# apache/datafusion-comet

Hardware: NVIDIA H100
Metric: rows/sec on TPC-H Q1 filter+agg (higher is better)
Workload: dtype i128

## Files before the change

### datafusion-comet_b200/csrc/abi.cpp

```cpp
#include "../../include/comet_b200.h"

#include "abi_internal.h"
#include "parquet_kernels.h"
#include "exec_internal.h"
#include "jit.h"
#include "plan.h"
#include "proto_wire.h"

#include <cstring>
#include <functional>
#include <map>
#include <mutex>

using namespace cb200;

namespace {

struct CtxRes {
    cudaStream_t stream;
    int* d_err;
    int* h_err;
    cudaEvent_t ev0, ev1;
};
std::mutex g_pool_mu;
// ... 27 lines not shown
    {
        struct DevInfo { int major = 0, minor = 0, sms = 0; bool known = false; };
        static DevInfo info[64];
        static std::mutex info_mu;
        std::lock_guard<std::mutex> lk(info_mu);
        if (ctx.device < 0 || ctx.device >= 64) throw ExecError(CB200_ERR_CUDA, "", "device ordinal out of range");
        DevInfo& di = info[ctx.device];
        if (!di.known) {
            cuda_check(cudaDeviceGetAttribute(&di.major, cudaDevAttrComputeCapabilityMajor, ctx.device), "cudaDeviceGetAttribute");
            cuda_check(cudaDeviceGetAttribute(&di.minor, cudaDevAttrComputeCapabilityMinor, ctx.device), "cudaDeviceGetAttribute");
            cuda_check(cudaDeviceGetAttribute(&di.sms, cudaDevAttrMultiProcessorCount, ctx.device), "cudaDeviceGetAttribute");
            di.known = true;
        }
        if (di.major != 9 || di.minor != 0) throw ExecError(CB200_ERR_CUDA, "", "comet_b200 kernels are built for sm_90a; device is sm_" + std::to_string(di.major * 10 + di.minor));
        ctx.num_sms = di.sms;
    }
    {
        std::lock_guard<std::mutex> lk(g_pool_mu);
        auto& fl = g_pool[ctx.device];
        if (!fl.empty()) {
            CtxRes r = fl.back();
            fl.pop_back();
            ctx.stream = r.stream; ctx.d_err = r.d_err; ctx.h_err = r.h_err; ctx.ev0 = r.ev0; ctx.ev1 = r.ev1;
        }
    }
    if (!ctx.stream) {
        cuda_check(cudaStreamCreateWithFlags(&ctx.stream, cudaStreamNonBlocking), "cudaStreamCreate");
        cudaMemPool_t pool;
        if (cudaDeviceGetDefaultMemPool(&pool, ctx.device) == cudaSuccess) {
            unsigned long long keep = ~0ull;
            cudaMemPoolSetAttribute(pool, cudaMemPoolAttrReleaseThreshold, &keep);
        }
        cuda_check(cudaMalloc((void**)&ctx.d_err, 64), "cudaMalloc err");
        cuda_check(cudaMallocHost((void**)&ctx.h_err, 64), "cudaMallocHost err");
        cuda_check(cudaEventCreate(&ctx.ev0), "cudaEventCreate");
        cuda_check(cudaEventCreate(&ctx.ev1), "cudaEventCreate");
    }
    cuda_check(cudaMemsetAsync(ctx.d_err, 0, 64, ctx.stream), "memset err");
    set_alloc_stream(ctx.stream);
    p->root = build_exec(p->op, &ctx, &p->inputs);
    p->started = true;
}

DType dtype_from_ids(int type_id, int precision, int scale) {
    if (type_id < 0 || type_id > 13) throw Unsupported("type id " + std::to_string(type_id));
    DType d;
    d.id = (TypeId)type_id;
    d.precision = precision;
    d.scale = scale;
    return d;
}

}

extern "C" {

const char* cb200_version(void) { return "comet_b200 0.1.0 (sm_90a; reference apache/datafusion-comet 1.1.0 @2699f59b)"; }

int cb200_supports(const uint8_t* op_proto, size_t op_len, cb200_error* why) {
    return cb200_guarded(why, [&]() -> int {
        OperatorP op = decode_plan(op_proto, op_len);
        plan_kernels_for_build(op);
        return 1;
    }, 0);
}

cb200_plan* cb200_create_plan(const uint8_t* op_proto, size_t op_len, const uint8_t* cfg_proto, size_t cfg_len, struct ArrowArrayStream** inputs,
// ... 329 lines not shown
```

### datafusion-comet_b200/csrc/agg.cpp

```cpp
#include "exec_internal.h"
#include "../../include/comet_b200.h"

#include "aot_kernels.h"
#include "ranges.h"

#include <algorithm>
#include <mutex>

namespace cb200 {

static std::mutex g_profile_mu;
static std::map<std::string, std::vector<int>> g_range_profile;

void reset_range_profiles() {
    std::lock_guard<std::mutex> lk(g_profile_mu);
    g_range_profile.clear();
}

namespace {

enum class Strategy { Undecided, Dense, Table, Stream };
enum Level { SAFE = 0, TYPE = 1, TIGHT = 2 };
constexpr int DENSE_MAX_GROUPS = 64;

// ... 42 lines not shown
            for (int k = (int)cards.size() - 1; k >= 0; k--) {
                int cd = code[(size_t)k];
                if (has_null[(size_t)k] && cd == cards[(size_t)k] - 1) cd = new_cards[(size_t)k] - 1;
                ng += cd * mul;
                mul *= new_cards[(size_t)k];
            }
            memcpy(&newt[(size_t)ng * n_words * 2], &oldt[(size_t)g * n_words * 2], (size_t)n_words * 16);
        }
        totals = host_to_device(newt.data(), newt.size() * 8, ctx, "regroup H2D");
        groups = new_groups;
    }

    void finalize(ExecContext* ctx, const Kernel& last, cb::FinParams fp, bool ungrouped, const std::vector<DType>& schema,
                  const std::vector<DictionaryP>& key_dicts, Batch& out) const {
        TraceSpan ts("agg.finalize");
        const GeneratedKernel& g = last.g;
        const int ng = groups;
        fp.totals = (cb::u64*)totals->ptr;
        fp.n_groups = ng;
        std::vector<size_t> off_v, off_n;
        size_t total_bytes = 0;
        auto take = [&](size_t n) { size_t o = total_bytes; total_bytes += (n + 15) / 16 * 16; return o; };
        for (size_t i = 0; i < g.out_cols.size(); i++) { off_v.push_back(take((size_t)ng * g.out_bytes[i])); off_n.push_back(take((size_t)ng)); }
        size_t off_present = take((size_t)ng);
        auto dbuf = std::make_shared<DeviceBuf>(total_bytes);
        for (size_t i = 0; i < g.out_cols.size(); i++) {
            fp.out[i] = (cb::u8*)dbuf->ptr + off_v[i];
            fp.outv[i] = (cb::u8*)dbuf->ptr + off_n[i];
        }
        fp.present = (cb::u8*)dbuf->ptr + off_present;
        void* args[] = {&fp};
        cuda_check(cudaLaunchKernel((const void*)last.mod->kernel(g.finalize_entry), dim3((ng + 127) / 128), dim3(128), args, 0, ctx->stream), "finalize launch");
        ctx->kernel_launches++;
        std::vector<uint8_t> hbuf(total_bytes);
        cuda_check(cudaMemcpyAsync(hbuf.data(), dbuf->ptr, total_bytes, cudaMemcpyDeviceToHost, ctx->stream), "agg results D2H"); ctx->d2h_bytes += (int64_t)(total_bytes);
        ctx->check_device_errors();
        const uint8_t* pres = hbuf.data() + off_present;
        std::vector<int> rows;
        for (int gi = 0; gi < ng; gi++) if (ungrouped || pres[(size_t)gi]) rows.push_back(gi);
        out.n_rows = (int64_t)rows.size();
        out.cols.clear();
        for (size_t k = 0; k < key_dicts.size(); k++) {
            Column c;
            c.type = schema[k];
            c.on_host = true;
            bool any_null = false;
            std::vector<int> codes;
            for (int gi : rows) codes.push_back(decode_gid(gi, cards)[k]);
            c.h_valid.assign(rows.size(), 1);
            const bool is_bool = c.type.id == TypeId::Bool;
            if (!is_bool) c.h_offsets.push_back(0);
            for (size_t r = 0; r < rows.size(); r++) {
                const bool isnull = has_null[k] && codes[r] == cards[k] - 1;
                if (isnull) { c.h_valid[r] = 0; any_null = true; }
                if (is_bool) c.h_data.push_back(isnull ? 0 : (uint8_t)codes[r]);
                else {
                    if (!isnull) { const std::string& s = key_dicts[k]->values().at((size_t)codes[r]); c.h_data.insert(c.h_data.end(), s.begin(), s.end()); }
                    c.h_offsets.push_back((int32_t)c.h_data.size());
                }
            }
            if (!any_null) c.h_valid.clear();
            out.cols.push_back(c);
        }
        for (size_t i = 0; i < g.out_cols.size(); i++) {
            Column c;
            c.type = g.out_cols[i].type;
            c.on_host = true;
            int w = g.out_bytes[i];
            const uint8_t* all = hbuf.data() + off_v[i];
            const uint8_t* allv = hbuf.data() + off_n[i];
            c.h_data.resize(rows.size() * w);
            c.h_valid.resize(rows.size());
            bool any_null = false;
            for (size_t r = 0; r < rows.size(); r++) {
                memcpy(&c.h_data[r * w], &all[(size_t)rows[r] * w], (size_t)w);
                c.h_valid[r] = allv[(size_t)rows[r]];
                if (!c.h_valid[r]) any_null = true;
            }
            if (!any_null) c.h_valid.clear();
            out.cols.push_back(c);
        }
    }
};

struct IdRows {
    DeviceBufP hkey_of_gid, htotals, hflags;
    int64_t max_groups = 0;

    void ensure_flags(ExecContext* ctx) {
        if (hflags) return;
        hflags = std::make_shared<DeviceBuf>(sizeof(HashFlags));
        cuda_check(cudaMemsetAsync(hflags->ptr, 0, sizeof(HashFlags), ctx->stream), "memset hash flags");
    }
    void write_flags(ExecContext* ctx, const HashFlags& hf) {
        cuda_check(cudaMemcpyAsync(hflags->ptr, &hf, sizeof(hf), cudaMemcpyHostToDevice, ctx->stream), "write hash flags");
        cuda_check(cudaStreamSynchronize(ctx->stream), "flags sync");
    }
    int64_t read_flags(ExecContext* ctx, HashFlags& hf, int64_t cnt[GK]) {
        memset(&hf, 0, sizeof(hf));
        if (hflags) {
            cuda_check(cudaMemcpyAsync(&hf, hflags->ptr, sizeof(hf), cudaMemcpyDeviceToHost, ctx->stream), "read hash flags"); ctx->d2h_bytes += (int64_t)sizeof(hf);
            cuda_check(cudaStreamSynchronize(ctx->stream), "hash flags sync");
        }
// ... 269 lines not shown
        Kernel k{spec, generate_pipeline(spec), nullptr};
        k.mod = jit_get(k.g, true);
        if (have_totals() && k.g.key_words != key_words) throw ExecError(15, "", "internal: group key packing changed between launches");
        if (have_totals() && (k.g.n_words != n_words || k.g.word_kinds != word_kinds || k.g.role_words != role_words)) widen(k);
        n_words = k.g.n_words;
        word_kinds = k.g.word_kinds;
        role_words = k.g.role_words;
        key_words = k.g.key_words;
        return k;
    }

    void widen(const Kernel& k) {
        GeneratedKernel from;
        from.n_words = n_words;
        from.word_kinds = word_kinds;
        from.role_words = role_words;
        const std::vector<int> map = widen_word_map(from, k.g);
        if (map.empty()) throw ExecError(15, "", "internal: accumulator layout changed between launches");
        const bool is_dense = strategy == Strategy::Dense;
        DeviceBufP& t = is_dense ? dense.totals : rows.htotals;
        const size_t n_rows = is_dense ? (size_t)dense.groups : (size_t)rows.max_groups + 2;
        auto nt = std::make_shared<DeviceBuf>(n_rows * (size_t)k.g.n_words * 16);
        for (int w = 0; w < k.g.n_words; w++)
            cuda_check(cudaMemcpy2DAsync((char*)nt->ptr + (size_t)w * 16, (size_t)k.g.n_words * 16, (const char*)t->ptr + (size_t)map[(size_t)w] * 16,
                                         (size_t)n_words * 16, 16, n_rows, cudaMemcpyDeviceToDevice, ctx->stream), "widen totals");
        cuda_check(cudaStreamSynchronize(ctx->stream), "widen totals");
        t = nt;
    }

    void clear_vmask() {
        if (!vmask) vmask = std::make_shared<DeviceBuf>(CB_MAX_COLS * 16);
        cuda_check(cudaMemsetAsync(vmask->ptr, 0, CB_MAX_COLS * 16, ctx->stream), "memset vmask");
    }
    void copy_vmask(ValueMasks& masks) {
        cuda_check(cudaMemcpyAsync(masks, vmask->ptr, sizeof(ValueMasks), cudaMemcpyDeviceToHost, ctx->stream), "read value masks"); ctx->d2h_bytes += (int64_t)(sizeof(ValueMasks));
    }
    static std::vector<int> mask_bits(const PipelineSpec& spec, const ValueMasks& masks) {
        std::vector<int> seen(spec.cols.size(), -1);
        for (size_t i = 0; i < spec.cols.size(); i++) {
            if (!spec.cols[i].type.is_decimal()) continue;
            uint64_t lo = masks[2 * i], hi = masks[2 * i + 1];
            seen[i] = hi ? 64 + r_bitlen(hi) : r_bitlen(lo);
        }
        return seen;
    }
    void observe(const std::vector<int>& seen) {
        for (size_t i = 0; i < seen.size(); i++)
            if (seen[i] >= 0) observed_bits[(size_t)used_cols[i]] = std::max(observed_bits[(size_t)used_cols[i]], seen[i]);
    }

    int prepare_key(Batch& b, size_t k) {
        int ci = keys[k]->index;
        Column& c = b.cols[ci];
        if (c.type.id == TypeId::Bool) return 2;
        if (!c.type.is_string()) return -1;
        if (c.is_dict) {
            key_dicts[k] = c.dict;
            return (int)c.dict->values().size();
        }
        if (!dev_dicts[k]) {
            auto dd = std::make_shared<DevDict>();
            const int64_t cap = 1 << 16;
            const int max_codes = 4096;
            const int64_t bytes_cap = 1 << 20;
            auto alloc = [&](size_t n) { auto bfr = std::make_shared<DeviceBuf>(n); cuda_check(cudaMemsetAsync(bfr->ptr, 0, bfr->bytes, ctx->stream), "memset dict"); dd->bufs.push_back(bfr); return bfr->ptr; };
            dd->d.tags = (unsigned long long*)alloc((size_t)cap * 8);
            dd->d.slot_code = (int*)alloc((size_t)cap * 4);
            dd->d.capacity = cap;
            dd->d.n_codes = (int*)alloc(64);
            dd->d.bytes_used = (unsigned long long*)((char*)dd->d.n_codes + 16);
            dd->d.err = (int*)((char*)dd->d.n_codes + 32);
            dd->d.max_codes = max_codes;
            dd->d.code_off = (long long*)alloc((size_t)max_codes * 8);
            dd->d.code_len = (int*)alloc((size_t)max_codes * 4);
            dd->d.bytes = (unsigned char*)alloc((size_t)bytes_cap);
            dd->d.bytes_cap = bytes_cap;
            dev_dicts[k] = dd;
            key_dicts[k] = std::make_shared<Dictionary>();
        }
        DevDict& dd = *dev_dicts[k];
        if (!c.offsets || !c.chars) throw Unsupported("string key column without offsets/chars buffers");
        auto row_slot = std::make_shared<DeviceBuf>((size_t)b.n_rows * 4);
        auto codes = std::make_shared<DeviceBuf>((size_t)b.n_rows * 4);
        launch_dict_encode(dd.d, (const int*)c.offsets->ptr, (const unsigned char*)c.chars->ptr, c.validity ? (const unsigned char*)c.validity->ptr : nullptr,
                           b.n_rows, (int*)row_slot->ptr, (int*)codes->ptr, ctx->stream);
        ctx->kernel_launches += 2;
        int hdr[12];
        cuda_check(cudaMemcpyAsync(hdr, dd.d.n_codes, sizeof(hdr), cudaMemcpyDeviceToHost, ctx->stream), "dict header");
        cuda_check(cudaStreamSynchronize(ctx->stream), "dict encode");
        int n_codes = hdr[0], derr = hdr[8];
        if (derr & CB_DICT_FULL) throw Unsupported("plain Utf8 group key with more distinct values than the device dictionary holds (dictionary-encode the column)");
        if (derr & CB_DICT_COLLISION) throw ExecError(14, "", "64-bit hash collision between distinct group key strings");
        if (n_codes > dd.host_known) {
            std::vector<long long> off((size_t)n_codes);
            std::vector<int> len((size_t)n_codes);
            cuda_check(cudaMemcpy(off.data(), dd.d.code_off, (size_t)n_codes * 8, cudaMemcpyDeviceToHost), "dict offsets");
            cuda_check(cudaMemcpy(len.data(), dd.d.code_len, (size_t)n_codes * 4, cudaMemcpyDeviceToHost), "dict lengths");
            for (int i = dd.host_known; i < n_codes; i++) {
                std::string s((size_t)len[(size_t)i], '\0');
                if (len[(size_t)i]) cuda_check(cudaMemcpy(&s[0], dd.d.bytes + off[(size_t)i], (size_t)len[(size_t)i], cudaMemcpyDeviceToHost), "dict bytes");
                key_dicts[k]->append(s);
            }
            dd.host_known = n_codes;
        }
        c.data = codes;
        c.phys = Phys::I32;
        c.is_dict = true;
        c.dict = key_dicts[k];
        return n_codes;
    }

    void consume(Batch& b) {
        for (int ci : used_cols) if (b.cols[(size_t)ci].validity) col_nullable[(size_t)ci] = true;
        std::vector<int> nc(keys.size());
        std::vector<bool> hn(keys.size());
        for (size_t k = 0; k < keys.size(); k++) {
            int card = prepare_key(b, k);
            const Column& c = b.cols[keys[k]->index];
            hn[k] = key_has_null[k] || c.validity != nullptr;
            nc[k] = card < 0 ? -1 : std::max(card, 1) + (hn[k] ? 1 : 0);
            if (!dense.cards.empty() && nc[k] >= 0) nc[k] = std::max(nc[k], dense.cards[k]);
        }
        bool densifiable = true;
        for (int c : nc) if (c < 0) densifiable = false;
        int n_groups = 1;
        if (densifiable) for (int c : nc) { n_groups *= c; if (n_groups > 1 << 20) break; }
        const bool needs_hash = !ungrouped && (!densifiable || n_groups > DENSE_MAX_GROUPS);
        key_has_null = hn;
        if (observed_bits.empty()) observed_bits.assign(child->schema.size(), -1);
        if (strategy == Strategy::Undecided || (strategy == Strategy::Dense && needs_hash)) {
            if (strategy == Strategy::Dense) {
                leave_dense();
                ctx->agg_strategies |= CB200_AGG_MIGRATED;
// ... 65 lines not shown
            while (r0 < row1 && launch_one(b, r0, std::min(row1, r0 + max_rows), n_groups, k, lv)) r0 += max_rows;
            if (r0 >= row1) return;
            if (lv == SAFE) throw ExecError(15, "", "internal: value-mask validation failed without assumptions");
            lv = lv == TIGHT ? TYPE : SAFE;
            row0 = r0;
        }
    }

    bool launch_one(Batch& b, int64_t r0, int64_t r1, int n_groups, const Kernel& k, Level lv) {
        cudaStream_t st = ctx->stream;
        size_t tot_bytes = (size_t)n_groups * n_words * 16;
        if (!have_totals()) {
            dense.totals = std::make_shared<DeviceBuf>(tot_bytes);
            dense.groups = n_groups;
        }
        if (!dense.spill || dense.spill->bytes < tot_bytes) {
            dense.spill = std::make_shared<DeviceBuf>(tot_bytes);
            cuda_check(cudaMemsetAsync(dense.spill->ptr, 0, dense.spill->bytes, st), "memset spill");
        }
        clear_vmask();
        cb::PipeParams p;
        fill_inputs(p, b, k.g.tile, r0, r1);
        bind_str_masks(p, k.spec, b);
        int grid = grid_for(ctx, p.n_tiles);
        size_t part_bytes = (size_t)grid * tot_bytes;
        if (!dense.partials || dense.partials->bytes < part_bytes) dense.partials = std::make_shared<DeviceBuf>(part_bytes);
        p.n_groups = n_groups;
        for (size_t i = 0; i < dense.cards.size() && i < CB_MAX_KEYS; i++) p.key_card[i] = dense.cards[i];
        p.partials = (cb::u8*)dense.partials->ptr;
        p.spill = (cb::u64*)dense.spill->ptr;
        p.vmask = (cb::u64*)vmask->ptr;
        launch(k.mod->kernel(k.g.entry), dim3(grid), dim3(k.g.threads + 32), k.g.dyn_smem(n_groups), &p);
        ctx->pipeline_rows += r1 - r0;
        ValueMasks masks;
        copy_vmask(masks);
        const int errs = ctx->take_device_errors();
        const std::vector<int> seen = mask_bits(k.spec, masks);
        bool ok = true;
        for (size_t i = 0; i < seen.size(); i++)
            if (k.spec.cols[i].assume_bits > 0 && seen[i] > k.spec.cols[i].assume_bits) ok = false;
        observe(seen);
        if (!ok) {
            cuda_check(cudaMemsetAsync(dense.spill->ptr, 0, dense.spill->bytes, st), "memset spill");
            ctx->agg_range_reruns++;
            return false;
        }
        ctx->raise_device_errors(errs);
        ctx->agg_range_levels |= lv == TIGHT ? CB200_RANGE_TIGHT : lv == TYPE ? CB200_RANGE_TYPE : CB200_RANGE_SAFE;
        rows_scanned += r1 - r0;
        cb::FinParams fp;
        memset(&fp, 0, sizeof(fp));
        fp.partials = (const cb::u64*)dense.partials->ptr;
        fp.spill = (cb::u64*)dense.spill->ptr;
        fp.totals = (cb::u64*)dense.totals->ptr;
        fp.n_ctas = grid;
        fp.n_groups = n_groups;
        fp.first = have_totals() ? 0 : 1;
        fp.err = ctx->d_err;
        int total_words = n_groups * n_words;
        void* args[] = {&fp};
        cuda_check(cudaLaunchKernel((const void*)k.mod->kernel("cb_fold"), dim3((total_words + 127) / 128), dim3(128), args, 0, st), "fold launch");
        ctx->kernel_launches++;
        last = k;
        return true;
    }

    void launch_id_rows(Batch& b, int64_t r0, int64_t r1, const Kernel& k, bool with_table) {
        clear_vmask();
        cb::PipeParams p;
        fill_inputs(p, b, k.g.tile, r0, r1);
        bind_str_masks(p, k.spec, b);
        p.hkeys = with_table ? (cb::u64*)table.hkeys->ptr : nullptr;
        p.hkey_of_gid = (cb::u64*)rows.hkey_of_gid->ptr;
        p.htotals = (cb::u64*)rows.htotals->ptr;
        p.hmask = with_table ? (cb::u32)(table.hcap - 1) : 0;
        p.max_groups = (cb::i32)rows.max_groups;
        p.hflags = (cb::i32*)rows.hflags->ptr;
        p.vmask = (cb::u64*)vmask->ptr;
        p.n_groups = 2;
        launch(k.mod->kernel(k.g.entry), dim3(grid_for(ctx, p.n_tiles)), dim3(k.g.threads + 32), k.g.dyn_smem(0), &p);
    }

    void consume_table(Batch& b) {
        const Kernel k = compile(make_spec(&b, Strategy::Table, 2, SAFE));
        {
            TraceSpan ts("hash.ensure_table");
            table.ensure(ctx, k, rows, b.n_rows, child->rows_hint(), rows_scanned, mode != AggMode::Partial || !all_partial);
        }
        launch_id_rows(b, 0, b.n_rows, k, true);
        ctx->pipeline_rows += b.n_rows;
        ValueMasks masks;
        int flags[8];
        copy_vmask(masks);
        cuda_check(cudaMemcpyAsync(flags, rows.hflags->ptr, sizeof(flags), cudaMemcpyDeviceToHost, ctx->stream), "read hash flags"); ctx->d2h_bytes += (int64_t)(sizeof(flags));
        ctx->check_device_errors();
        if (flags[0] & CB_HF_FULL) throw ExecError(15, "", "internal: hash table full");
        if (flags[0] & CB_HF_WIDE_KEY) throw Unsupported("decimal(p > 18) group key whose value does not fit 64 bits");
        observe(mask_bits(k.spec, masks));
        rows_scanned += b.n_rows;
        last = k;
    }

    int64_t stream_launch(Batch& b, int64_t r0, int64_t r1, const Kernel& k, HashFlags& hf, int64_t cnt[GK]) {
        launch_id_rows(b, r0, r1, k, false);
        ValueMasks masks;
        copy_vmask(masks);
        ctx->check_device_errors();
        const int64_t total = rows.read_flags(ctx, hf, cnt);
        if (hf.w[0] & CB_HF_WIDE_KEY) throw Unsupported("decimal(p > 18) group key whose value does not fit 64 bits");
        if (!(hf.w[0] & CB_HF_FULL)) observe(mask_bits(k.spec, masks));
        return total;
    }
    bool sample_stream(Batch& b) {
        if (mode != AggMode::Partial || !all_partial || ctx->stream_agg_min_rows < 0) return false;
        if (b.n_rows + std::max<int64_t>(child->rows_hint(), 0) < ctx->stream_agg_min_rows || b.n_rows == 0) return false;
        const Kernel k = compile(make_spec(&b, Strategy::Stream, 2, SAFE));
        const int64_t sample = std::min<int64_t>(b.n_rows, 1 << 20);
        HashFlags hf;
        int64_t cnt[GK] = {0};
        stream.ensure_rows(ctx, k, rows, cnt, 2 * sample + 4096);
        const int64_t runs = stream_launch(b, 0, sample, k, hf, cnt);
        stream.ratio = (hf.w[0] & CB_HF_FULL) ? 1.0 : (double)runs / (double)sample;
        memset(&hf, 0, sizeof(hf));
        rows.write_flags(ctx, hf);
        IdRows::init_totals(ctx, k, (cb::u64*)rows.htotals->ptr, rows.max_groups, 2);
        if (stream.ratio <= ctx->stream_agg_max_ratio) return true;
        rows = IdRows();
        n_words = 0; word_kinds.clear(); role_words.clear();
        return false;
    }
    void consume_stream(Batch& b) {
        const Kernel k = compile(make_spec(&b, Strategy::Stream, 2, SAFE));
        HashFlags before, hf;
        int64_t cnt0[GK], cnt[GK];
        const int64_t cur = rows.read_flags(ctx, before, cnt0);
        const int64_t remaining = std::max<int64_t>(child->rows_hint(), 0);
        int64_t want = cur + std::min<int64_t>(b.n_rows, (int64_t)(1.25 * stream.ratio * (double)b.n_rows) + 65536);
        if (!rows.htotals || want > rows.max_groups) want += std::min<int64_t>(remaining, (int64_t)(1.25 * stream.ratio * (double)remaining));
        int64_t handed_out;
        while (true) {
// ... 137 lines not shown
```

### datafusion-comet_b200/csrc/codegen.cpp

```cpp
#include "codegen.h"
#include <mutex>
#include "device/cb_params.h"
#include "ranges.h"

#include <algorithm>
#include <climits>
#include <cstring>
#include <functional>
#include <memory>
#include <set>
#include <sstream>

namespace cb200 {

int phys_bytes(Phys p) {
    switch (p) {
    case Phys::Bitmap: return 0;
    case Phys::I8: return 1;
    case Phys::I16: return 2;
    case Phys::I32: case Phys::F32: case Phys::Dict32: return 4;
    case Phys::I64: case Phys::F64: return 8;
    case Phys::I128: return 16;
    }
    return 0;
}

size_t GeneratedKernel::dyn_smem(int n_groups) const {
    size_t s = (entry == "cb_pipeline_agg" ? 128 : 256) + (size_t)stages * stage_bytes;
    if (hash) return s;
    if (!word_kinds.empty() && !ungrouped) s += (size_t)std::max(n_groups, 1) * n_words * threads * 8;
    return s;
}

namespace {

struct Val {
    std::string v;
    std::string n;
    DType type;
    bool narrow = false;
    bool nullable() const { return !n.empty(); }
};
const u128r R63 = (u128r)1 << 63;

// ... 639 lines not shown
    return b;
}

int out_width(const DType& t) { return t.id == TypeId::Bool ? 1 : t.arrow_width(); }

int key_bits(const DType& t) {
    switch (t.id) {
    case TypeId::Bool: return 1;
    case TypeId::Int8: return 8;
    case TypeId::Int16: return 16;
    case TypeId::Int32: case TypeId::Date: return 32;
    case TypeId::String: return 32;
    case TypeId::Int64: case TypeId::Timestamp: case TypeId::TimestampNtz: return 64;
    case TypeId::Decimal: return t.precision <= 18 ? 64 : 0;
    default: return 0;
    }
}

std::string to_slot(const Val& v, const std::string& dst) {
    const DType& t = v.type;
    std::ostringstream o;
    if (t.is_decimal() && v.narrow) o << dst << "[0] = (cb::u64)" << v.v << "; " << dst << "[1] = (cb::u64)(" << v.v << " >> 63);";
    else if (t.is_decimal()) o << dst << "[0] = " << v.v << ".lo; " << dst << "[1] = (cb::u64)" << v.v << ".hi;";
    else if (t.id == TypeId::Float64) o << dst << "[0] = (cb::u64)__double_as_longlong(" << v.v << ");";
    else if (t.id == TypeId::Float32) o << dst << "[0] = (cb::u64)__float_as_uint(" << v.v << ");";
    else if (t.id == TypeId::Bool) o << dst << "[0] = " << v.v << " ? 1ull : 0ull;";
    else o << dst << "[0] = (cb::u64)(cb::i64)" << v.v << ";";
    return o.str();
}

}

namespace {
void sig_expr(std::ostringstream& o, const Expr& e) {
    uint64_t fb;
    memcpy(&fb, &e.lit_f64, 8);
    o << (int)e.kind << '|' << e.type.str() << '|' << e.index << '|' << e.lit_null << '|' << e.lit_i64 << '|' << fb << '|' << (uint64_t)e.lit_dec << ','
      << (uint64_t)(e.lit_dec >> 64) << '|' << e.lit_str << '|' << (int)e.eval_mode << '|' << e.fail_on_error << '|' << e.negated << '|' << e.wide_decimal << '|' << e.integral_div << e.check_divide_overflow << '|'
      << e.return_type.str() << '(';
    if (e.kind == ExprKind::StrPred) o << str_pred_key(e) << '|' << e.in_has_null << '|';
    for (auto& c : e.children) { sig_expr(o, *c); o << ','; }
    o << ')';
}
std::string spec_signature(const PipelineSpec& s) {
    std::ostringstream o;
    o << (int)s.sink << ';' << (int)s.mode << ';' << s.ungrouped << ';' << s.hash << (s.stream ? "s" : "") << (s.masked ? "m" : "") << ';' << s.tile << ';' << s.stages << ';' << s.threads << ';' << s.ltile << ";C";
    for (auto& c : s.cols) o << c.src_index << ':' << c.type.str() << ':' << (int)c.phys << ':' << c.has_validity << ':' << c.assume_bits << (c.layout_nullable && !c.has_validity ? "L" : "") << ',';
    o << ";P";
    for (auto& e : s.predicates) { sig_expr(o, *e); o << ';'; }
    o << ";O";
    for (auto& e : s.outputs) { sig_expr(o, *e); o << ';'; }
    o << ";K";
    for (size_t i = 0; i < s.keys.size(); i++) { sig_expr(o, *s.keys[i]); o << (i < s.key_nullable.size() && s.key_nullable[i]) << ';'; }
    o << ";A";
    for (auto& a : s.aggs) {
        o << (int)a.kind << ':' << (int)a.mode << ':' << a.datatype.str() << ':' << a.sum_datatype.str() << ':' << (int)a.eval_mode << '[';
        for (auto& c : a.children) { sig_expr(o, *c); o << ','; }
        o << "]F";
        if (a.filter) sig_expr(o, *a.filter);
        o << ';';
    }
    o << ";S";
    for (auto& v : s.state_slots) { for (int x : v) o << x << ','; o << ';'; }
    return o.str();
}
std::mutex g_memo_mu;
std::map<std::string, GeneratedKernel> g_memo;
GeneratedKernel generate_pipeline_uncached(const PipelineSpec& spec);
}

std::string pipeline_signature(const PipelineSpec& spec) { return spec_signature(spec); }

std::vector<int> widen_word_map(const GeneratedKernel& from, const GeneratedKernel& to) {
    if (from.role_words.size() != to.role_words.size()) return {};
    std::vector<int> map((size_t)to.n_words, -1);
    auto set = [&](int w, int o) {
        if (map[(size_t)w] >= 0 && map[(size_t)w] != o) return false;
        map[(size_t)w] = o;
        return true;
    };
    for (size_t r = 0; r < to.role_words.size(); r++) {
        const int w = to.role_words[r], o = from.role_words[r];
        if ((w < 0) != (o < 0)) return {};
        if (w < 0) continue;
        if (!set(w, o)) return {};
        if (to.word_kinds[(size_t)w] == W_DD_HI && !set(w + 1, o + 1)) return {};
    }
    for (int w = 0; w < to.n_words; w++)
        if (map[(size_t)w] < 0 || from.word_kinds.at((size_t)map[(size_t)w]) != to.word_kinds[(size_t)w]) return {};
    return map;
}

std::string str_pred_key(const Expr& e) {
    std::ostringstream o;
    o << (int)e.str_op << ':' << e.str_lits.size();
    for (auto& l : e.str_lits) o << ':' << l.size() << '=' << l;
    return o.str();
// ... 579 lines not shown
```

### datafusion-comet_b200/csrc/exec.cpp

```cpp
#include "exec_internal.h"

#include <cstdlib>
#include <ctime>
#include <mutex>

namespace cb200 {

enum { ERR_I128_OVERFLOW = 0, ERR_ANSI_OVERFLOW = 1, ERR_ORDER_DEPENDENT = 2, ERR_DIVIDE_BY_ZERO = 3, ERR_ARROW_DIVIDE_BY_ZERO = 4, ERR_DICT_CODE = 5,
       ERR_WIDE_MINMAX = 6 };

bool trace_on() {
    static int on = -1;
    if (on < 0) { const char* e = getenv("CB200_TRACE"); on = (e && *e && *e != '0') ? 1 : 0; }
    return on == 1;
}
double now_ms() {
    struct timespec ts;
    clock_gettime(CLOCK_MONOTONIC, &ts);
    return ts.tv_sec * 1e3 + ts.tv_nsec * 1e-6;
}
TraceSpan::TraceSpan(const char* n) : name(n), t0(trace_on() ? now_ms() : 0) {}
TraceSpan::~TraceSpan() {
    if (trace_on()) { static const double tz = now_ms(); const double t1 = now_ms(); fprintf(stderr, "[cb200 trace] %-28s %8.3f ms   (ends at +%.3f ms)\n", name, t1 - t0, t1 - tz); }
}
// ... 265 lines not shown
                col_is_dict[i] = true;
                dict_index_width[i] = it.arrow_width();
                if (it.arrow_width() == 8) throw Unsupported("int64 dictionary indices");
                dicts[i] = std::make_shared<Dictionary>();
            } else {
                DType t = dtype_from_format(ch->format);
                bool ok = t == schema[i] || (t.is_decimal() && schema[i].is_decimal() && t.scale == schema[i].scale) ||
                          (t.id == TypeId::Timestamp && schema[i].id == TypeId::TimestampNtz) || (t.id == TypeId::TimestampNtz && schema[i].id == TypeId::Timestamp);
                if (!ok) throw PlanError("scan field " + std::to_string(i) + " is " + schema[i].str() + " but the stream column is " + t.str());
            }
        }
        if (sc.release) sc.release(&sc);
        schema_checked = true;
    }

    bool next(Batch& out) override {
        if (!schema_checked) check_schema();
        if (eof) return false;
        std::vector<ArrowArray> arrs;
        int64_t total = 0;
        while (total < ctx->chunk_rows) {
            ArrowArray a;
            memset(&a, 0, sizeof(a));
            if (stream->get_next(stream, &a) != 0) {
                const char* m = stream->get_last_error ? stream->get_last_error(stream) : nullptr;
                for (auto& x : arrs) if (x.release) x.release(&x);
                throw ExecError(3, "", std::string("ArrowArrayStream get_next failed: ") + (m ? m : "?"));
            }
            if (!a.release) { eof = true; break; }
            if (a.length > 0) { total += a.length; arrs.push_back(a); }
            else a.release(&a);
        }
        if (arrs.empty()) return false;
        try {
            upload(arrs, total, out);
        } catch (...) {
            for (auto& x : arrs) if (x.release) x.release(&x);
            throw;
        }
        cuda_check(cudaStreamSynchronize(ctx->stream), "H2D copies");
        for (auto& x : arrs) if (x.release) x.release(&x);
        return true;
    }

    std::vector<int32_t> unify_dict(size_t col, const ArrowArray* d) {
        Dictionary& g = *dicts[col];
        const int32_t* off = (const int32_t*)d->buffers[1] + d->offset;
        const char* chars = (const char*)d->buffers[2];
        std::vector<int32_t> remap((size_t)d->length);
        bool identity = true;
        for (int64_t k = 0; k < d->length; k++) {
            const int32_t code = g.intern(std::string(chars + off[k], (size_t)(off[k + 1] - off[k])));
            remap[(size_t)k] = code;
            if (code != k) identity = false;
        }
        if (identity) remap.clear();
        return remap;
    }

    cudaError_t h2d(void* dst, const void* src, size_t n) {
        ctx->h2d_bytes += (int64_t)n;
        return cudaMemcpyAsync(dst, src, n, cudaMemcpyHostToDevice, ctx->stream);
    }

    void upload(std::vector<ArrowArray>& arrs, int64_t total, Batch& out) {
        TraceSpan ts("source.upload");
        out.n_rows = total;
        out.cols.clear();
        out.cols.resize(schema.size());
        cudaStream_t st = ctx->stream;
        for (size_t c = 0; c < schema.size(); c++) {
            Column& col = out.cols[c];
            col.type = schema[c];
            bool any_nulls = false;
            for (auto& a : arrs) {
                ArrowArray* ch = a.children[c];
                if (ch->null_count != 0 && ch->buffers[0]) any_nulls = true;
            }
            if (any_nulls) {
                col.validity = std::make_shared<DeviceBuf>((size_t)(total + 7) / 8 + 8);
                cuda_check(cudaMemsetAsync(col.validity->ptr, 0, col.validity->bytes, st), "memset validity");
            }
            std::vector<DeviceBufP> temps;
            if (col_is_dict[c]) {
                col.is_dict = true;
                col.dict = dicts[c];
                int w = dict_index_width[c];
                bool need_remap = false;
                std::vector<std::vector<int32_t>> remaps;
                for (auto& a : arrs) {
                    remaps.push_back(unify_dict(c, a.children[c]->dictionary));
                    if (!remaps.back().empty()) need_remap = true;
                }
                if (!need_remap) {
                    col.phys = w == 1 ? Phys::I8 : w == 2 ? Phys::I16 : Phys::I32;
                    col.data = std::make_shared<DeviceBuf>((size_t)total * w);
                } else {
                    col.phys = Phys::I32;
                    col.data = std::make_shared<DeviceBuf>((size_t)total * 4);
                }
                int64_t row = 0;
                for (size_t k = 0; k < arrs.size(); k++) {
                    ArrowArray* ch = arrs[k].children[c];
                    const char* src = (const char*)ch->buffers[1] + ch->offset * w;
                    if (!need_remap) {
                        cuda_check(h2d((char*)col.data->ptr + row * w, src, (size_t)ch->length * w), "H2D dict codes");
                    } else {
                        auto tmp = std::make_shared<DeviceBuf>((size_t)ch->length * w);
                        temps.push_back(tmp);
                        cuda_check(h2d(tmp->ptr, src, (size_t)ch->length * w), "H2D dict codes");
                        std::vector<int32_t> table = remaps[k];
                        if (table.empty()) { table.resize((size_t)ch->dictionary->length); for (size_t i = 0; i < table.size(); i++) table[i] = (int32_t)i; }
                        DeviceBufP dt = host_to_device(table.data(), table.size() * 4, ctx, "H2D remap table");
                        ctx->h2d_bytes += (int64_t)(table.size() * 4);
                        temps.push_back(dt);
                        launch_remap_codes(tmp->ptr, w, ch->length, (const int*)dt->ptr, (int)table.size(), (int*)col.data->ptr + row, st);
                    }
                    row += ch->length;
                }
            } else if (schema[c].is_string()) {
                int64_t total_chars = 0;
                for (auto& a : arrs) {
                    ArrowArray* ch = a.children[c];
                    const int32_t* off = (const int32_t*)ch->buffers[1] + ch->offset;
                    total_chars += off[ch->length] - off[0];
                }
                if (total_chars > INT32_MAX) throw Unsupported("more than 2 GiB of string data in one chunk");
                col.chars = std::make_shared<DeviceBuf>((size_t)total_chars + 16);
                std::vector<int32_t> offs((size_t)total + 1);
                int64_t row = 0;
                int32_t base = 0;
                for (auto& a : arrs) {
                    ArrowArray* ch = a.children[c];
                    const int32_t* off = (const int32_t*)ch->buffers[1] + ch->offset;
                    for (int64_t i = 0; i < ch->length; i++) offs[(size_t)(row + i)] = base + (off[i] - off[0]);
                    int32_t nchars = off[ch->length] - off[0];
                    if (nchars) cuda_check(h2d((char*)col.chars->ptr + base, (const char*)ch->buffers[2] + off[0], (size_t)nchars), "H2D chars");
                    base += nchars;
                    row += ch->length;
                }
                offs[(size_t)total] = base;
                col.offsets = host_to_device(offs.data(), offs.size() * 4, ctx, "H2D offsets");
                ctx->h2d_bytes += (int64_t)(offs.size() * 4);
                col.phys = Phys::I32;
            } else {
                col.phys = phys_of(schema[c]);
                int w = schema[c].arrow_width();
                if (w == 0) {
                    col.data = std::make_shared<DeviceBuf>((size_t)(total + 7) / 8 + 8);
                    cuda_check(cudaMemsetAsync(col.data->ptr, 0, col.data->bytes, st), "memset bool");
                    int64_t row = 0;
                    for (auto& a : arrs) {
                        ArrowArray* ch = a.children[c];
                        append_bits((uint32_t*)col.data->ptr, row, (const uint8_t*)ch->buffers[1], ch->offset, ch->length, temps);
                        row += ch->length;
                    }
                } else {
                    col.data = std::make_shared<DeviceBuf>((size_t)total * w);
                    int64_t row = 0;
                    for (auto& a : arrs) {
                        ArrowArray* ch = a.children[c];
                        cuda_check(h2d((char*)col.data->ptr + row * w, (const char*)ch->buffers[1] + ch->offset * w, (size_t)ch->length * w), "H2D column");
                        row += ch->length;
                    }
                }
            }
            if (any_nulls) {
                int64_t row = 0, nulls = 0;
                for (auto& a : arrs) {
                    ArrowArray* ch = a.children[c];
                    bool has = ch->null_count != 0 && ch->buffers[0];
                    append_bits((uint32_t*)col.validity->ptr, row, has ? (const uint8_t*)ch->buffers[0] : nullptr, ch->offset, ch->length, temps);
                    nulls += has ? (ch->null_count < 0 ? 1 : ch->null_count) : 0;
                    row += ch->length;
                }
                col.null_count = nulls;
            }
            if (!temps.empty()) cuda_check(cudaStreamSynchronize(st), "temp buffers");
        }
    }

    void append_bits(uint32_t* dst, int64_t row, const uint8_t* src, int64_t src_off, int64_t n, std::vector<DeviceBufP>& temps) {
        if (n <= 0) return;
        if (src && (row & 7) == 0 && (src_off & 7) == 0 && ((n & 7) == 0)) {
            cuda_check(h2d((char*)dst + (row >> 3), src + (src_off >> 3), (size_t)(n >> 3)), "H2D bitmap");
            return;
        }
        const uint8_t* dsrc = nullptr;
        int64_t doff = 0;
        if (src) {
            int64_t b0 = src_off >> 3, b1 = (src_off + n + 7) >> 3;
            auto tmp = std::make_shared<DeviceBuf>((size_t)(b1 - b0) + 8);
            temps.push_back(tmp);
            cuda_check(h2d(tmp->ptr, src + b0, (size_t)(b1 - b0)), "H2D bitmap");
            dsrc = (const uint8_t*)tmp->ptr;
            doff = src_off & 7;
        }
        launch_bitmap_append(dst, row, dsrc, doff, n, ctx->stream);
    }
};

struct TableSource : ExecNode {
    std::shared_ptr<DeviceTable> table;
    ExecContext* ctx = nullptr;
    bool done = false;
    TableSource(std::shared_ptr<DeviceTable> t, const std::vector<DType>& fields, ExecContext* c) : table(std::move(t)), ctx(c) {
        schema = fields;
        if (table->cols.size() != fields.size()) throw PlanError("bound device table has " + std::to_string(table->cols.size()) + " columns, scan declares " + std::to_string(fields.size()));
    }
    int64_t pos = 0;
    bool packed = false;
// ... 449 lines not shown
```

### datafusion-comet_b200/csrc/exec.h

```cpp
#pragma once
#include "arrow_abi.h"
#include "codegen.h"
#include "jit.h"
#include "plan.h"

#include <cuda_runtime.h>
#include <climits>
#include <memory>
#include <string>
#include <unordered_map>
#include <vector>

namespace cb200 {

struct ExecError : std::runtime_error {
    int code;
    std::string error_class;
    ExecError(int c, const std::string& cls, const std::string& msg) : std::runtime_error(msg), code(c), error_class(cls) {}
};

void cuda_check(cudaError_t e, const char* what);

struct TraceSpan {
    const char* name;
// ... 51 lines not shown

struct Column {
    DType type;
    Phys phys = Phys::I32;
    bool is_dict = false;
    DictionaryP dict;
    DeviceBufP data, validity;
    DeviceBufP offsets, chars;
    DeviceBufP valid_bytes;
    DeviceBufP bool_bytes;
    int64_t null_count = 0;
    bool on_host = false;
    std::vector<uint8_t> h_data;
    std::vector<uint8_t> h_valid;
    std::vector<int32_t> h_offsets;
};

struct Batch {
    int64_t n_rows = 0;
    std::vector<Column> cols;
};

struct ExecContext {
    int device = 0;
    cudaStream_t stream = nullptr;
    int num_sms = 132;
    int64_t chunk_rows = 1ll << 26;
    int hash_threads = 512;
    int64_t stream_agg_min_rows = 4 << 20;
    double stream_agg_max_ratio = 0.5;
    int batch_size = 8192;
    int* d_err = nullptr;
    int* h_err = nullptr;
    int64_t kernel_launches = 0;
    cudaEvent_t ev0 = nullptr, ev1 = nullptr;
    bool ev_pending = false;
    double pipeline_ms = 0;
    int64_t pipeline_launches = 0;
    int64_t pipeline_rows = 0;
    int64_t h2d_bytes = 0, d2h_bytes = 0;
    int64_t scan_pruned_row_groups = 0, scan_pruned_rows = 0;
    int64_t scan_pruned_pages = 0, scan_page_pruned_rows = 0;
    int64_t agg_strategies = 0;
    int64_t agg_range_levels = 0;
    int64_t agg_range_reruns = 0;
    int64_t sort_rows = 0, sort_passes = 0, sort_pass_rows = 0;
    int64_t sort_select_rows = 0;
    int64_t join_build_rows = 0, join_probe_rows = 0, join_out_rows = 0;
    int64_t join_cond_pairs = 0;
    double partition_ids_ms = 0, partition_place_ms = 0, partition_gather_ms = 0;
    int64_t agg_table_grows = 0;
    int64_t agg_stream_reruns = 0;
    std::vector<int64_t> partition_starts;
    void check_device_errors() { raise_device_errors(take_device_errors()); }
    int take_device_errors();
    void raise_device_errors(int e);
    void collect_timing();
};

struct ExecNode {
    std::vector<DType> schema;
    virtual ~ExecNode() {}
    virtual bool next(Batch& out) = 0;
    virtual std::vector<std::shared_ptr<ExecNode>> children() const { return {}; }
    virtual std::vector<PipelineSpec> build_specs() const { return {}; }
    virtual void push_filters(const std::vector<ExprP>&) {}
// ... 28 lines not shown
```

Measured before the change: 39.19 billion.

## Use pinned scratch for small readbacks, batch dict allocations, speed up signatures

Adds a pinned host scratch region after the error word and uses it for the aggregate result, value-mask and dictionary header copies, replacing pageable host buffers. Dictionary device buffers are folded into one allocation and one memset, and the first 64 codes and their bytes are read back speculatively to avoid follow-up synchronous copies. Kernel signature strings are built with to_chars instead of ostringstream, and source upload no longer synchronizes per column on temporary buffers. The main risks are aliasing of the shared scratch between back-to-back readbacks and temporaries now living until the end of the upload.

```diff
diff --git a/datafusion-comet_b200/csrc/abi.cpp b/datafusion-comet_b200/csrc/abi.cpp
--- a/datafusion-comet_b200/csrc/abi.cpp
+++ b/datafusion-comet_b200/csrc/abi.cpp
@@ -83,7 +83,7 @@
             cudaMemPoolSetAttribute(pool, cudaMemPoolAttrReleaseThreshold, &keep);
         }
         cuda_check(cudaMalloc((void**)&ctx.d_err, 64), "cudaMalloc err");
-        cuda_check(cudaMallocHost((void**)&ctx.h_err, 64), "cudaMallocHost err");
+        cuda_check(cudaMallocHost((void**)&ctx.h_err, ExecContext::PINNED_SCRATCH_BYTES), "cudaMallocHost err");
         cuda_check(cudaEventCreate(&ctx.ev0), "cudaEventCreate");
         cuda_check(cudaEventCreate(&ctx.ev1), "cudaEventCreate");
     }
diff --git a/datafusion-comet_b200/csrc/agg.cpp b/datafusion-comet_b200/csrc/agg.cpp
--- a/datafusion-comet_b200/csrc/agg.cpp
+++ b/datafusion-comet_b200/csrc/agg.cpp
@@ -98,10 +98,12 @@
         void* args[] = {&fp};
         cuda_check(cudaLaunchKernel((const void*)last.mod->kernel(g.finalize_entry), dim3((ng + 127) / 128), dim3(128), args, 0, ctx->stream), "finalize launch");
         ctx->kernel_launches++;
-        std::vector<uint8_t> hbuf(total_bytes);
-        cuda_check(cudaMemcpyAsync(hbuf.data(), dbuf->ptr, total_bytes, cudaMemcpyDeviceToHost, ctx->stream), "agg results D2H"); ctx->d2h_bytes += (int64_t)(total_bytes);
+        std::vector<uint8_t> pageable;
+        if (total_bytes > ExecContext::pinned_scratch_bytes()) pageable.resize(total_bytes);
+        uint8_t* const hres = pageable.empty() ? ctx->pinned_scratch() : pageable.data();
+        cuda_check(cudaMemcpyAsync(hres, dbuf->ptr, total_bytes, cudaMemcpyDeviceToHost, ctx->stream), "agg results D2H"); ctx->d2h_bytes += (int64_t)(total_bytes);
         ctx->check_device_errors();
-        const uint8_t* pres = hbuf.data() + off_present;
+        const uint8_t* pres = hres + off_present;
         std::vector<int> rows;
         for (int gi = 0; gi < ng; gi++) if (ungrouped || pres[(size_t)gi]) rows.push_back(gi);
         out.n_rows = (int64_t)rows.size();
@@ -133,8 +135,8 @@
             c.type = g.out_cols[i].type;
             c.on_host = true;
             int w = g.out_bytes[i];
-            const uint8_t* all = hbuf.data() + off_v[i];
-            const uint8_t* allv = hbuf.data() + off_n[i];
+            const uint8_t* all = hres + off_v[i];
+            const uint8_t* allv = hres + off_n[i];
             c.h_data.resize(rows.size() * w);
             c.h_valid.resize(rows.size());
             bool any_null = false;
@@ -470,9 +472,11 @@
         if (!vmask) vmask = std::make_shared<DeviceBuf>(CB_MAX_COLS * 16);
         cuda_check(cudaMemsetAsync(vmask->ptr, 0, CB_MAX_COLS * 16, ctx->stream), "memset vmask");
     }
-    void copy_vmask(ValueMasks& masks) {
-        cuda_check(cudaMemcpyAsync(masks, vmask->ptr, sizeof(ValueMasks), cudaMemcpyDeviceToHost, ctx->stream), "read value masks"); ctx->d2h_bytes += (int64_t)(sizeof(ValueMasks));
-    }
+    void copy_vmask() {
+        static_assert(sizeof(ValueMasks) <= ExecContext::pinned_scratch_bytes(), "value masks exceed the pinned scratch");
+        cuda_check(cudaMemcpyAsync(ctx->pinned_scratch(), vmask->ptr, sizeof(ValueMasks), cudaMemcpyDeviceToHost, ctx->stream), "read value masks"); ctx->d2h_bytes += (int64_t)(sizeof(ValueMasks));
+    }
+    void read_vmask(ValueMasks& masks) const { memcpy(masks, ctx->pinned_scratch(), sizeof(ValueMasks)); }
     static std::vector<int> mask_bits(const PipelineSpec& spec, const ValueMasks& masks) {
         std::vector<int> seen(spec.cols.size(), -1);
         for (size_t i = 0; i < spec.cols.size(); i++) {
@@ -501,17 +505,24 @@
             const int64_t cap = 1 << 16;
             const int max_codes = 4096;
             const int64_t bytes_cap = 1 << 20;
-            auto alloc = [&](size_t n) { auto bfr = std::make_shared<DeviceBuf>(n); cuda_check(cudaMemsetAsync(bfr->ptr, 0, bfr->bytes, ctx->stream), "memset dict"); dd->bufs.push_back(bfr); return bfr->ptr; };
-            dd->d.tags = (unsigned long long*)alloc((size_t)cap * 8);
-            dd->d.slot_code = (int*)alloc((size_t)cap * 4);
+            size_t at = 0;
+            auto part = [&](size_t n) { size_t o = at; at += (n + 255) / 256 * 256; return o; };
+            const size_t o_tags = part((size_t)cap * 8), o_slot = part((size_t)cap * 4), o_hdr = part(64), o_off = part((size_t)max_codes * 8),
+                         o_len = part((size_t)max_codes * 4), o_bytes = part((size_t)bytes_cap);
+            auto blk = std::make_shared<DeviceBuf>(at);
+            cuda_check(cudaMemsetAsync(blk->ptr, 0, blk->bytes, ctx->stream), "memset dict");
+            dd->bufs.push_back(blk);
+            char* base = (char*)blk->ptr;
+            dd->d.tags = (unsigned long long*)(base + o_tags);
+            dd->d.slot_code = (int*)(base + o_slot);
             dd->d.capacity = cap;
-            dd->d.n_codes = (int*)alloc(64);
+            dd->d.n_codes = (int*)(base + o_hdr);
             dd->d.bytes_used = (unsigned long long*)((char*)dd->d.n_codes + 16);
             dd->d.err = (int*)((char*)dd->d.n_codes + 32);
             dd->d.max_codes = max_codes;
-            dd->d.code_off = (long long*)alloc((size_t)max_codes * 8);
-            dd->d.code_len = (int*)alloc((size_t)max_codes * 4);
-            dd->d.bytes = (unsigned char*)alloc((size_t)bytes_cap);
+            dd->d.code_off = (long long*)(base + o_off);
+            dd->d.code_len = (int*)(base + o_len);
+            dd->d.bytes = (unsigned char*)(base + o_bytes);
             dd->d.bytes_cap = bytes_cap;
             dev_dicts[k] = dd;
             key_dicts[k] = std::make_shared<Dictionary>();
@@ -523,20 +534,39 @@
         launch_dict_encode(dd.d, (const int*)c.offsets->ptr, (const unsigned char*)c.chars->ptr, c.validity ? (const unsigned char*)c.validity->ptr : nullptr,
                            b.n_rows, (int*)row_slot->ptr, (int*)codes->ptr, ctx->stream);
         ctx->kernel_launches += 2;
-        int hdr[12];
-        cuda_check(cudaMemcpyAsync(hdr, dd.d.n_codes, sizeof(hdr), cudaMemcpyDeviceToHost, ctx->stream), "dict header");
-        cuda_check(cudaStreamSynchronize(ctx->stream), "dict encode");
+        constexpr int HDR = 12, SPEC_CODES = 64;
+        constexpr size_t SPEC_BYTES = 4096;
+        uint8_t* const pin = ctx->pinned_scratch();
+        int* const hdr = (int*)pin;
+        long long* const spec_off = (long long*)(pin + 64);
+        int* const spec_len = (int*)(pin + 64 + SPEC_CODES * 8);
+        const uint8_t* const spec_bytes = pin + 64 + SPEC_CODES * 12;
+        static_assert(64 + SPEC_CODES * 12 + SPEC_BYTES <= ExecContext::pinned_scratch_bytes(), "dictionary read-back exceeds the pinned scratch");
+        cudaStream_t st = ctx->stream;
+        cuda_check(cudaMemcpyAsync(hdr, dd.d.n_codes, HDR * sizeof(int), cudaMemcpyDeviceToHost, st), "dict header");
+        cuda_check(cudaMemcpyAsync(spec_off, dd.d.code_off, SPEC_CODES * 8, cudaMemcpyDeviceToHost, st), "dict offsets");
+        cuda_check(cudaMemcpyAsync(spec_len, dd.d.code_len, SPEC_CODES * 4, cudaMemcpyDeviceToHost, st), "dict lengths");
+        cuda_check(cudaMemcpyAsync((void*)spec_bytes, dd.d.bytes, SPEC_BYTES, cudaMemcpyDeviceToHost, st), "dict bytes");
+        cuda_check(cudaStreamSynchronize(st), "dict encode");
         int n_codes = hdr[0], derr = hdr[8];
         if (derr & CB_DICT_FULL) throw Unsupported("plain Utf8 group key with more distinct values than the device dictionary holds (dictionary-encode the column)");
         if (derr & CB_DICT_COLLISION) throw ExecError(14, "", "64-bit hash collision between distinct group key strings");
         if (n_codes > dd.host_known) {
+            bool have = n_codes <= SPEC_CODES;
+            for (int i = dd.host_known; have && i < n_codes; i++) have = spec_off[i] >= 0 && (size_t)spec_off[i] + (size_t)spec_len[i] <= SPEC_BYTES;
             std::vector<long long> off((size_t)n_codes);
             std::vector<int> len((size_t)n_codes);
-            cuda_check(cudaMemcpy(off.data(), dd.d.code_off, (size_t)n_codes * 8, cudaMemcpyDeviceToHost), "dict offsets");
-            cuda_check(cudaMemcpy(len.data(), dd.d.code_len, (size_t)n_codes * 4, cudaMemcpyDeviceToHost), "dict lengths");
+            if (have) {
+                memcpy(off.data(), spec_off, (size_t)n_codes * 8);
+                memcpy(len.data(), spec_len, (size_t)n_codes * 4);
+            } else {
+                cuda_check(cudaMemcpy(off.data(), dd.d.code_off, (size_t)n_codes * 8, cudaMemcpyDeviceToHost), "dict offsets");
+                cuda_check(cudaMemcpy(len.data(), dd.d.code_len, (size_t)n_codes * 4, cudaMemcpyDeviceToHost), "dict lengths");
+            }
             for (int i = dd.host_known; i < n_codes; i++) {
                 std::string s((size_t)len[(size_t)i], '\0');
-                if (len[(size_t)i]) cuda_check(cudaMemcpy(&s[0], dd.d.bytes + off[(size_t)i], (size_t)len[(size_t)i], cudaMemcpyDeviceToHost), "dict bytes");
+                if (len[(size_t)i] && have) memcpy(&s[0], spec_bytes + off[(size_t)i], (size_t)len[(size_t)i]);
+                else if (len[(size_t)i]) cuda_check(cudaMemcpy(&s[0], dd.d.bytes + off[(size_t)i], (size_t)len[(size_t)i], cudaMemcpyDeviceToHost), "dict bytes");
                 key_dicts[k]->append(s);
             }
             dd.host_known = n_codes;
@@ -668,9 +698,10 @@
         p.vmask = (cb::u64*)vmask->ptr;
         launch(k.mod->kernel(k.g.entry), dim3(grid), dim3(k.g.threads + 32), k.g.dyn_smem(n_groups), &p);
         ctx->pipeline_rows += r1 - r0;
+        copy_vmask();
+        const int errs = ctx->take_device_errors();
         ValueMasks masks;
-        copy_vmask(masks);
-        const int errs = ctx->take_device_errors();
+        read_vmask(masks);
         const std::vector<int> seen = mask_bits(k.spec, masks);
         bool ok = true;
         for (size_t i = 0; i < seen.size(); i++)
@@ -727,9 +758,10 @@
         ctx->pipeline_rows += b.n_rows;
         ValueMasks masks;
         int flags[8];
-        copy_vmask(masks);
+        copy_vmask();
         cuda_check(cudaMemcpyAsync(flags, rows.hflags->ptr, sizeof(flags), cudaMemcpyDeviceToHost, ctx->stream), "read hash flags"); ctx->d2h_bytes += (int64_t)(sizeof(flags));
         ctx->check_device_errors();
+        read_vmask(masks);
         if (flags[0] & CB_HF_FULL) throw ExecError(15, "", "internal: hash table full");
         if (flags[0] & CB_HF_WIDE_KEY) throw Unsupported("decimal(p > 18) group key whose value does not fit 64 bits");
         observe(mask_bits(k.spec, masks));
@@ -740,8 +772,9 @@
     int64_t stream_launch(Batch& b, int64_t r0, int64_t r1, const Kernel& k, HashFlags& hf, int64_t cnt[GK]) {
         launch_id_rows(b, r0, r1, k, false);
         ValueMasks masks;
-        copy_vmask(masks);
+        copy_vmask();
         ctx->check_device_errors();
+        read_vmask(masks);
         const int64_t total = rows.read_flags(ctx, hf, cnt);
         if (hf.w[0] & CB_HF_WIDE_KEY) throw Unsupported("decimal(p > 18) group key whose value does not fit 64 bits");
         if (!(hf.w[0] & CB_HF_FULL)) observe(mask_bits(k.spec, masks));
diff --git a/datafusion-comet_b200/csrc/codegen.cpp b/datafusion-comet_b200/csrc/codegen.cpp
--- a/datafusion-comet_b200/csrc/codegen.cpp
+++ b/datafusion-comet_b200/csrc/codegen.cpp
@@ -4,12 +4,14 @@
 #include "ranges.h"
 
 #include <algorithm>
+#include <charconv>
 #include <climits>
 #include <cstring>
 #include <functional>
 #include <memory>
 #include <set>
 #include <sstream>
+#include <type_traits>
 
 namespace cb200 {
 
@@ -715,20 +717,39 @@
 }
 
 namespace {
-void sig_expr(std::ostringstream& o, const Expr& e) {
+struct SigOut {
+    std::string s;
+    SigOut& operator<<(char c) { s += c; return *this; }
+    SigOut& operator<<(const char* c) { s += c; return *this; }
+    SigOut& operator<<(const std::string& c) { s += c; return *this; }
+    SigOut& operator<<(bool b) { s += b ? '1' : '0'; return *this; }
+    SigOut& operator<<(const DType& t) {
+        if (t.id != TypeId::Decimal) return *this << t.str();
+        return *this << "decimal128(" << t.precision << ',' << t.scale << ')';
+    }
+    template <typename T, typename = std::enable_if_t<std::is_integral_v<T>>>
+    SigOut& operator<<(T v) {
+        char b[24];
+        const auto r = std::to_chars(b, b + sizeof(b), v);
+        s.append(b, r.ptr);
+        return *this;
+    }
+};
+void sig_expr(SigOut& o, const Expr& e) {
     uint64_t fb;
     memcpy(&fb, &e.lit_f64, 8);
-    o << (int)e.kind << '|' << e.type.str() << '|' << e.index << '|' << e.lit_null << '|' << e.lit_i64 << '|' << fb << '|' << (uint64_t)e.lit_dec << ','
+    o << (int)e.kind << '|' << e.type << '|' << e.index << '|' << e.lit_null << '|' << e.lit_i64 << '|' << fb << '|' << (uint64_t)e.lit_dec << ','
       << (uint64_t)(e.lit_dec >> 64) << '|' << e.lit_str << '|' << (int)e.eval_mode << '|' << e.fail_on_error << '|' << e.negated << '|' << e.wide_decimal << '|' << e.integral_div << e.check_divide_overflow << '|'
-      << e.return_type.str() << '(';
+      << e.return_type << '(';
     if (e.kind == ExprKind::StrPred) o << str_pred_key(e) << '|' << e.in_has_null << '|';
     for (auto& c : e.children) { sig_expr(o, *c); o << ','; }
     o << ')';
 }
 std::string spec_signature(const PipelineSpec& s) {
-    std::ostringstream o;
+    SigOut o;
+    o.s.reserve(4096);
     o << (int)s.sink << ';' << (int)s.mode << ';' << s.ungrouped << ';' << s.hash << (s.stream ? "s" : "") << (s.masked ? "m" : "") << ';' << s.tile << ';' << s.stages << ';' << s.threads << ';' << s.ltile << ";C";
-    for (auto& c : s.cols) o << c.src_index << ':' << c.type.str() << ':' << (int)c.phys << ':' << c.has_validity << ':' << c.assume_bits << (c.layout_nullable && !c.has_validity ? "L" : "") << ',';
+    for (auto& c : s.cols) o << c.src_index << ':' << c.type << ':' << (int)c.phys << ':' << c.has_validity << ':' << c.assume_bits << (c.layout_nullable && !c.has_validity ? "L" : "") << ',';
     o << ";P";
     for (auto& e : s.predicates) { sig_expr(o, *e); o << ';'; }
     o << ";O";
@@ -737,7 +758,7 @@
     for (size_t i = 0; i < s.keys.size(); i++) { sig_expr(o, *s.keys[i]); o << (i < s.key_nullable.size() && s.key_nullable[i]) << ';'; }
     o << ";A";
     for (auto& a : s.aggs) {
-        o << (int)a.kind << ':' << (int)a.mode << ':' << a.datatype.str() << ':' << a.sum_datatype.str() << ':' << (int)a.eval_mode << '[';
+        o << (int)a.kind << ':' << (int)a.mode << ':' << a.datatype << ':' << a.sum_datatype << ':' << (int)a.eval_mode << '[';
         for (auto& c : a.children) { sig_expr(o, *c); o << ','; }
         o << "]F";
         if (a.filter) sig_expr(o, *a.filter);
@@ -745,7 +766,7 @@
     }
     o << ";S";
     for (auto& v : s.state_slots) { for (int x : v) o << x << ','; o << ';'; }
-    return o.str();
+    return std::move(o.s);
 }
 std::mutex g_memo_mu;
 std::map<std::string, GeneratedKernel> g_memo;
diff --git a/datafusion-comet_b200/csrc/exec.cpp b/datafusion-comet_b200/csrc/exec.cpp
--- a/datafusion-comet_b200/csrc/exec.cpp
+++ b/datafusion-comet_b200/csrc/exec.cpp
@@ -321,8 +321,9 @@
             else a.release(&a);
         }
         if (arrs.empty()) return false;
+        std::vector<DeviceBufP> temps;
         try {
-            upload(arrs, total, out);
+            upload(arrs, total, out, temps);
         } catch (...) {
             for (auto& x : arrs) if (x.release) x.release(&x);
             throw;
@@ -352,7 +353,7 @@
         return cudaMemcpyAsync(dst, src, n, cudaMemcpyHostToDevice, ctx->stream);
     }
 
-    void upload(std::vector<ArrowArray>& arrs, int64_t total, Batch& out) {
+    void upload(std::vector<ArrowArray>& arrs, int64_t total, Batch& out, std::vector<DeviceBufP>& temps) {
         TraceSpan ts("source.upload");
         out.n_rows = total;
         out.cols.clear();
@@ -370,7 +371,6 @@
                 col.validity = std::make_shared<DeviceBuf>((size_t)(total + 7) / 8 + 8);
                 cuda_check(cudaMemsetAsync(col.validity->ptr, 0, col.validity->bytes, st), "memset validity");
             }
-            std::vector<DeviceBufP> temps;
             if (col_is_dict[c]) {
                 col.is_dict = true;
                 col.dict = dicts[c];
@@ -429,8 +429,8 @@
                     row += ch->length;
                 }
                 offs[(size_t)total] = base;
-                col.offsets = host_to_device(offs.data(), offs.size() * 4, ctx, "H2D offsets");
-                ctx->h2d_bytes += (int64_t)(offs.size() * 4);
+                col.offsets = std::make_shared<DeviceBuf>(offs.size() * 4);
+                cuda_check(h2d(col.offsets->ptr, offs.data(), offs.size() * 4), "H2D offsets");
                 col.phys = Phys::I32;
             } else {
                 col.phys = phys_of(schema[c]);
@@ -465,7 +465,6 @@
                 }
                 col.null_count = nulls;
             }
-            if (!temps.empty()) cuda_check(cudaStreamSynchronize(st), "temp buffers");
         }
     }
 
diff --git a/datafusion-comet_b200/csrc/exec.h b/datafusion-comet_b200/csrc/exec.h
--- a/datafusion-comet_b200/csrc/exec.h
+++ b/datafusion-comet_b200/csrc/exec.h
@@ -107,6 +107,9 @@
     int batch_size = 8192;
     int* d_err = nullptr;
     int* h_err = nullptr;
+    static constexpr size_t PINNED_SCRATCH_BYTES = 16384;
+    uint8_t* pinned_scratch() const { return (uint8_t*)h_err + 64; }
+    static constexpr size_t pinned_scratch_bytes() { return PINNED_SCRATCH_BYTES - 64; }
     int64_t kernel_launches = 0;
     cudaEvent_t ev0 = nullptr, ev1 = nullptr;
     bool ev_pending = false;
```

Measured after the change: 40.87 billion (median of 6 runs). 4.3% higher.
